# Eden-Kramer-Lab/spectral_connectivity

Hardware: AMD Instinct MI355X
Metric: channel-pair*freq-bins/s for CSM+coherence(+wPLI) (higher is better)
Workload: dtype f32

## Files before the change

### spectral_connectivity_amd/csrc/sc_api.hip

```cpp
#include <stdarg.h>
#include <stdlib.h>
#include <string.h>
#include <rocfft/rocfft.h>
#include "sc_common.h"

static thread_local char g_err[512] = "";

void sc_set_error(const char* fmt, ...) {
    va_list ap;
    va_start(ap, fmt);
    vsnprintf(g_err, sizeof(g_err), fmt, ap);
    va_end(ap);
}

static const char* const g_switch_names[SC_SW_COUNT] = {
    "SC_FUSED_DEBUG", "SC_FUSED2_TERMS", "SC_FUSED_SPLIT", "SC_FUSED_NO_SMALL", "SC_MTFFT_DEBUG", "SC_MTFFT_WIDE", "SC_MTFFT_F64",
    "SC_F64_SPLIT", "SC_F64_OC", "SC_F64_NO_FORK", "SC_F64_NO_BLOCK", "SC_WILSON_FFT", "SC_GLOBAL_EIG", "SC_GLOBAL_NT256",
    "SC_GRANGER_KERNEL", "SC_FUSED_FOLD_OBS", "SC_MTFFT_LONG", "SC_CANON_EIG", "SC_MTFFT_MIXED", "SC_MTFFT_MIXED_GEO", "SC_MTFFT_SLICE", "SC_MVAR_INVERSE"};
static char g_switch_val[SC_SW_COUNT][32];
static bool g_switch_set[SC_SW_COUNT];
extern "C" int sc_debug_reload_env(void) {
    for (int i = 0; i < SC_SW_COUNT; ++i) {
        const char* v = getenv(g_switch_names[i]);
        g_switch_set[i] = v != nullptr;
        if (v) { strncpy(g_switch_val[i], v, sizeof(g_switch_val[i]) - 1); g_switch_val[i][sizeof(g_switch_val[i]) - 1] = 0; }
    }
    return SC_OK;
}
static const int g_switches_loaded = sc_debug_reload_env();
const char* sc_switch(int id) { return (id >= 0 && id < SC_SW_COUNT && g_switch_set[id]) ? g_switch_val[id] : nullptr; }

#include <mutex>
#include <vector>
struct ScZ2zEntry { int type; size_t N, batch; rocfft_plan plan; };
static std::vector<ScZ2zEntry> g_z2z;
static std::mutex g_z2z_mutex;
static int64_t g_plans_created = 0;
int sc_internal_z2z_plan(rocfft_plan* plan, int forward, size_t N, size_t batch, bool* cached) {
    std::lock_guard<std::mutex> lock(g_z2z_mutex);
    for (const ScZ2zEntry& e : g_z2z)
        if (e.type == forward && e.N == N && e.batch == batch) { *plan = e.plan; *cached = true; return SC_OK; }
    size_t lengths[1] = {N};
    const rocfft_status s = rocfft_plan_create(plan, rocfft_placement_inplace,
                                               forward ? rocfft_transform_type_complex_forward : rocfft_transform_type_complex_inverse,
                                               rocfft_precision_double, 1, lengths, batch, nullptr);
    if (s != rocfft_status_success) {
        sc_set_error("rocfft_plan_create(Z2Z N=%zu batch=%zu) failed: %d", N, batch, (int)s);
        return SC_EFFT;
    }
    ++g_plans_created;
    *cached = true;
    g_z2z.push_back(ScZ2zEntry{forward, N, batch, *plan});
    return SC_OK;
}

struct ScR2cEntry { int64_t N, rows; int f64; rocfft_plan plan; bool busy; };
static std::vector<ScR2cEntry> g_r2c;
static rocfft_plan r2c_pool_take(int64_t N, int64_t rows, bool f64) {
    std::lock_guard<std::mutex> lock(g_z2z_mutex);
    for (ScR2cEntry& e : g_r2c)
        if (!e.busy && e.N == N && e.rows == rows && e.f64 == (f64 ? 1 : 0)) { e.busy = true; return e.plan; }
    return nullptr;
}
static void r2c_pool_add(int64_t N, int64_t rows, bool f64, rocfft_plan plan) {
    std::lock_guard<std::mutex> lock(g_z2z_mutex);
    ++g_plans_created;
    g_r2c.push_back(ScR2cEntry{N, rows, f64 ? 1 : 0, plan, true});
}
static void r2c_pool_release(rocfft_plan plan) {
    if (!plan) return;
    std::lock_guard<std::mutex> lock(g_z2z_mutex);
    for (ScR2cEntry& e : g_r2c)
        if (e.plan == plan) { e.busy = false; return; }
}
extern "C" int sc_debug_fft_plans(int64_t* n_created, int64_t* n_pooled, int64_t* n_idle) {
    std::lock_guard<std::mutex> lock(g_z2z_mutex);
    int64_t idle = 0;
    for (const ScR2cEntry& e : g_r2c) idle += e.busy ? 0 : 1;
    if (n_created) *n_created = g_plans_created;
    if (n_pooled) *n_pooled = (int64_t)(g_r2c.size() + g_z2z.size());
    if (n_idle) *n_idle = idle;
    return SC_OK;
}

extern "C" int sc_abi_version(void) { return SC_ABI_VERSION; }
extern "C" const char* sc_last_error(void) { return g_err; }

extern "C" int sc_device_count(int* count) {
    SC_REQUIRE(count != nullptr, "count is NULL");
    int n = 0;
    hipError_t e = hipGetDeviceCount(&n);
    if (e != hipSuccess) { (void)hipGetLastError(); n = 0; }
    *count = n;
    return SC_OK;
}

struct sc_fft_plan {
    rocfft_plan plan, tail_plan;
    rocfft_execution_info info;
    void* work;
    void* Z;
    size_t work_bytes;
    int64_t N, batch, chunk, tail;
    int f64;
};

static int g_rocfft_ready = 0;

#define SC_CHECK_FFT(expr)                                                          \
    do {                                                                            \
        rocfft_status s_ = (expr);                                                  \
        if (s_ != rocfft_status_success) {                                          \
            sc_set_error("%s failed: rocfft_status %d (%s:%d)", #expr, (int)s_,     \
                         __FILE__, __LINE__);                                       \
            return SC_EFFT;                                                         \
        }                                                                           \
    } while (0)

static int make_r2c_rows(rocfft_plan* plan, int64_t N, int64_t rows, bool f64) {
    if ((*plan = r2c_pool_take(N, rows, f64)) != nullptr) return SC_OK;
    rocfft_plan_description desc = nullptr;
    SC_CHECK_FFT(rocfft_plan_description_create(&desc));
    size_t one[1] = {1};
    const size_t F = (size_t)(N / 2 + 1);
    SC_CHECK_FFT(rocfft_plan_description_set_data_layout(
        desc, rocfft_array_type_real, rocfft_array_type_hermitian_interleaved, nullptr, nullptr,
        1, one, (size_t)N, 1, one, F));
    size_t lengths[1] = {(size_t)N};
    const rocfft_status s = rocfft_plan_create(plan, rocfft_placement_notinplace, rocfft_transform_type_real_forward,
                                               f64 ? rocfft_precision_double : rocfft_precision_single, 1, lengths,
                                               (size_t)rows, desc);
    rocfft_plan_description_destroy(desc);
    if (s != rocfft_status_success) {
        sc_set_error("rocfft_plan_create(N=%lld, rows=%lld) failed: status %d", (long long)N, (long long)rows, (int)s);
        *plan = nullptr;
        return SC_EFFT;
    }
    r2c_pool_add(N, rows, f64, *plan);
    return SC_OK;
}

extern "C" int sc_fft_plan_destroy(sc_fft_plan* plan);

static int fft_plan_create(sc_fft_plan** out, int64_t N, int64_t batch, bool f64) {
    SC_REQUIRE(out != nullptr, "plan out pointer is NULL");
    SC_REQUIRE(N >= 1 && batch >= 1, "N and batch must be positive");
    if (!g_rocfft_ready) { SC_CHECK_FFT(rocfft_setup()); g_rocfft_ready = 1; }
    sc_fft_plan* p = new sc_fft_plan();
    memset(p, 0, sizeof(*p));
    p->N = N; p->batch = batch; p->f64 = f64 ? 1 : 0;
    const int64_t F = N / 2 + 1;
    const size_t zsize = f64 ? sizeof(double2) : sizeof(float2);
    int64_t chunk = ((int64_t)(64u << 20) / (F * (int64_t)zsize)) & ~(int64_t)63;
    if (chunk < 64) chunk = 64;
    if (chunk > batch) chunk = batch;
    p->chunk = chunk;
    p->tail = batch % chunk;
    int rc = make_r2c_rows(&p->plan, N, chunk, f64);
    if (rc == SC_OK && p->tail) rc = make_r2c_rows(&p->tail_plan, N, p->tail, f64);
    if (rc != SC_OK) { sc_fft_plan_destroy(p); return rc; }
    size_t w1 = 0, w2 = 0;
    if (rocfft_plan_get_work_buffer_size(p->plan, &w1) != rocfft_status_success ||
        (p->tail_plan && rocfft_plan_get_work_buffer_size(p->tail_plan, &w2) != rocfft_status_success) ||
        rocfft_execution_info_create(&p->info) != rocfft_status_success) {
        sc_set_error("rocFFT work-buffer query failed (N=%lld)", (long long)N);
        sc_fft_plan_destroy(p);
        return SC_EFFT;
    }
    p->work_bytes = w1 > w2 ? w1 : w2;
    if ((p->work_bytes && hipMalloc(&p->work, p->work_bytes) != hipSuccess) ||
        hipMalloc((void**)&p->Z, (size_t)chunk * F * zsize) != hipSuccess) {
// ... 116 lines not shown
```

### spectral_connectivity_amd/csrc/sc_common.h

```cpp
#pragma once
#include <hip/hip_runtime.h>
#include <stdint.h>
#include <stdio.h>
#include "../../include/sc_hip.h"

void sc_set_error(const char* fmt, ...);

enum ScSwitch {
    SC_SW_FUSED_DEBUG, SC_SW_FUSED2_TERMS, SC_SW_FUSED_SPLIT, SC_SW_FUSED_NO_SMALL, SC_SW_MTFFT_DEBUG, SC_SW_MTFFT_WIDE,
    SC_SW_MTFFT_F64, SC_SW_F64_SPLIT, SC_SW_F64_OC, SC_SW_F64_NO_FORK, SC_SW_F64_NO_BLOCK, SC_SW_WILSON_FFT, SC_SW_GLOBAL_EIG,
    SC_SW_GLOBAL_NT256, SC_SW_GRANGER_KERNEL, SC_SW_FUSED_FOLD_OBS, SC_SW_MTFFT_LONG, SC_SW_CANON_EIG, SC_SW_MTFFT_MIXED, SC_SW_MTFFT_MIXED_GEO, SC_SW_MTFFT_SLICE, SC_SW_MVAR_INVERSE, SC_SW_COUNT
};
const char* sc_switch(int id);

int sc_internal_rows_to_bins(const void* d_Z, void* d_X, int64_t rows, int64_t F, int64_t batch, int64_t b_off,
                             int64_t nyquist_row, hipStream_t st);

bool sc_internal_mtfft_long_applies(int64_t N, int64_t C, int64_t groups);
int64_t sc_internal_mtfft_long_coverage(int64_t N, int64_t C);
int sc_internal_mtfft_long(const float* d_x, int64_t T, int64_t R, int64_t C, int64_t L, int64_t step, int64_t W, int64_t N,
                           const float* d_tapers, int64_t K, int detrend_type, const void* d_twiddles, void* d_X, void* d_P,
                           const float* d_scale, hipStream_t st);

bool sc_internal_mtfft_mix_has(int64_t N);
bool sc_internal_mtfft_mix_applies(int64_t N, int64_t C, int64_t groups);
int64_t sc_internal_mtfft_mix_coverage(int64_t N, int64_t C, bool planes);
int sc_internal_mtfft_mix(const float* d_x, int64_t T, int64_t R, int64_t C, int64_t L, int64_t step, int64_t W, int64_t N,
                          const float* d_tapers, int64_t K, int detrend_type, const void* d_twiddles, void* d_X, void* d_P,
                          const float* d_scale, hipStream_t st);

struct rocfft_plan_t;
int sc_internal_z2z_plan(struct rocfft_plan_t** plan, int forward, size_t N, size_t batch, bool* cached);

bool sc_internal_causal_fft_supported(int64_t N);
bool sc_internal_causal_fft_natural_supported(int64_t N);
int sc_internal_causal_fft_pair_natural(void* d_A, const int32_t* d_status, int64_t n_problems, int C, int64_t N,
                                        hipStream_t st);
int sc_internal_causal_fft_pair(void* d_A, const int32_t* d_status, int64_t n_problems, int C, int64_t N,
                                hipStream_t st);

bool sc_internal_granger_resident_applies(int64_t n_freq_accum, int64_t N);
int sc_internal_granger_resident(const void* d_accum, int64_t n_groups, int64_t N, int64_t C, uint32_t planes, int64_t n_obs,
                                 const int32_t* d_pairs, int64_t n_pairs, double tol, int max_iter, void* d_work, size_t work_bytes,
                                 int keep_output, double* d_out, int32_t* d_n_iter, int32_t* d_status, int32_t* h_summary,
                                 hipStream_t st);

int sc_internal_mvar_inverse(int64_t C, int64_t P, int64_t N, int64_t n_bins, const void* d_M, void* d_out, void* scratch,
                             const double* d_zero, hipStream_t st);
int sc_internal_mvar_gemm(int64_t C, int64_t n_problems, int64_t n_bins, const void* X, int64_t x_sp, int64_t x_sn,
                          const void* Y, int64_t y_sp, int64_t y_sn, void* O, int64_t o_sp, int64_t o_sn, hipStream_t st);

struct ScTimed {
    int slot;
    void* st;
    ScTimed(const char* name, void* stream);
    ~ScTimed();
    ScTimed(const ScTimed&) = delete;
    ScTimed& operator=(const ScTimed&) = delete;
};

#define SC_CHECK_HIP(expr)                                                        \
    do {                                                                          \
        hipError_t e_ = (expr);                                                   \
        if (e_ != hipSuccess) {                                                   \
            sc_set_error("%s failed: %s (%s:%d)", #expr, hipGetErrorString(e_),   \
                         __FILE__, __LINE__);                                     \
            return SC_EHIP;                                                       \
        }                                                                         \
    } while (0)

#define SC_REQUIRE(cond, msg)                                                     \
    do {                                                                          \
        if (!(cond)) {                                                            \
            sc_set_error("invalid argument: %s (%s)", msg, #cond);                \
            return SC_EINVAL;                                                     \
        }                                                                         \
    } while (0)

struct ScRec {
    const void* p;
    int f64;
    __host__ __device__ ScRec operator+(int64_t n) const { return ScRec{(const char*)p + n * (f64 ? 8 : 4), f64}; }
    __device__ double operator[](int64_t i) const {
        return f64 ? ((const double*)p)[i] : (double)((const float*)p)[i];
    }
};
__host__ inline ScRec sc_rec(const void* d_accum, uint32_t planes) { return ScRec{d_accum, (planes & SC_RECORD_F64) ? 1 : 0}; }

#define SC_TILE 16
#define SC_TILE_ELEMS 256
#define SC_MAX_SIGNALS 256

__host__ __device__ inline int sc_plane_count(uint32_t planes) {
    int n = 0;
    if (planes & SC_PLANE_CSM) n += 2;
    if (planes & SC_PLANE_ABS_IM) n += 1;
    if (planes & SC_PLANE_IM_SQ) n += 1;
    if (planes & SC_PLANE_SIGN_IM) n += 1;
    if (planes & SC_PLANE_UNIT) n += 2;
    return n;
}
__host__ __device__ inline int sc_plane_offset(uint32_t planes, uint32_t which) {
    int n = 0;
    if (which == SC_PLANE_CSM) return n;
    if (planes & SC_PLANE_CSM) n += 2;
    if (which == SC_PLANE_ABS_IM) return n;
    if (planes & SC_PLANE_ABS_IM) n += 1;
    if (which == SC_PLANE_IM_SQ) return n;
    if (planes & SC_PLANE_IM_SQ) n += 1;
    if (which == SC_PLANE_SIGN_IM) return n;
    if (planes & SC_PLANE_SIGN_IM) n += 1;
    return n;
}
__host__ __device__ inline int sc_n_blocks(int64_t C) { return (int)((C + SC_TILE - 1) / SC_TILE); }
__host__ __device__ inline int sc_n_tiles(int nb) { return nb * (nb + 1) / 2; }
__host__ __device__ inline int sc_tile_index(int bi, int bj, int nb) {
    return bi * nb - bi * (bi - 1) / 2 + (bj - bi);
}

struct ScCsmView {
    int64_t N, F, floats_per_bin;
    int NB, n_tiles, p_csm, two_sided;
    double n_obs;
};
inline int sc_csm_view(uint32_t planes, int64_t n_freq_accum, int64_t N, int64_t C, int64_t n_obs, ScCsmView* v) {
    SC_REQUIRE(planes & SC_PLANE_CSM, "accumulator record must contain SC_PLANE_CSM");
    SC_REQUIRE(n_freq_accum == N || n_freq_accum == N / 2 + 1, "accumulators must hold N or N/2+1 bins");
    SC_REQUIRE(n_obs >= 1, "n_observations must be positive");
    v->N = N; v->F = n_freq_accum;
    v->NB = sc_n_blocks(C); v->n_tiles = sc_n_tiles(v->NB);
    v->p_csm = sc_plane_offset(planes, SC_PLANE_CSM);
    v->two_sided = n_freq_accum == N ? 1 : 0;
    v->floats_per_bin = (int64_t)sc_plane_count(planes) * v->n_tiles * SC_TILE_ELEMS;
    v->n_obs = (double)n_obs;
    return SC_OK;
}
__device__ inline double2 sc_csm_two_sided(ScRec accum, const ScCsmView& v, int64_t g, int64_t n, int i, int j) {
    int64_t bin = n;
    bool conj = false;
    if (!v.two_sided && n > v.N / 2) { bin = v.N - n; conj = true; }
    const ScRec rec = accum + (g * v.F + bin) * v.floats_per_bin;
    int ti = i >> 4, tj = j >> 4, ii = i & 15, jj = j & 15;
    const bool m = (ti > tj) || (ti == tj && ii > jj);
    if (m) { int t = ti; ti = tj; tj = t; t = ii; ii = jj; jj = t; }
    const int64_t off = (int64_t)sc_tile_index(ti, tj, v.NB) * SC_TILE_ELEMS + ii * 16 + jj;
    const double re = rec[(int64_t)v.p_csm * v.n_tiles * SC_TILE_ELEMS + off] / v.n_obs;
    double im = rec[(int64_t)(v.p_csm + 1) * v.n_tiles * SC_TILE_ELEMS + off] / v.n_obs;
    if (m) im = -im;
    if (conj) im = -im;
    if (i == j) im = 0.0;
    return make_double2(re, im);
}

__device__ inline void sc_wg_cholesky(double2* L, int ld, int n, int* bad) {
    const int tid = threadIdx.x;
    for (int k = 0; k < n; ++k) {
        if (tid == 0) {
            const double d = L[k * ld + k].x;
            if (!(d > 0.0)) *bad = 1;
            L[k * ld + k] = make_double2(sqrt(d > 0.0 ? d : 1.0), 0.0);
        }
        __syncthreads();
        const double dk = L[k * ld + k].x;
        for (int i = k + 1 + tid; i < n; i += 256) {
// ... 78 lines not shown
```

### spectral_connectivity_amd/csrc/sc_mtfft_long.hip

```cpp
#include <cstdlib>
#include <type_traits>
#include "sc_common.h"
#include "sc_mtfft_bfly.h"

struct LongArgs {
    const float* x;
    const float* tapers;
    const float2* tw;
    float2* X;
    int R, C, L, step, W, K, detrend;
    int n_items;
    int g_off, g_end;
    int vec;
    unsigned char* P;
    const float* scale;
    int64_t row_bytes;
    int dbg;
};

typedef _Float16 ml_h16x2 __attribute__((ext_vector_type(2)));
typedef unsigned ml_u32x4 __attribute__((ext_vector_type(4)));
typedef unsigned ml_u32x2 __attribute__((ext_vector_type(2)));
__device__ __forceinline__ void ml_split2(float x0, float x1, unsigned& h, unsigned& m) {
    asm("v_cvt_pk_f16_f32 %0, %1, %2" : "=v"(h) : "v"(x0), "v"(x1));
    asm("v_fma_mixlo_f16 %0, %1, 1.0, -%2 op_sel_hi:[0,0,1]" : "=v"(m) : "v"(x0), "v"(h));
    asm("v_fma_mixhi_f16 %0, %1, 1.0, -%2 op_sel:[0,0,1] op_sel_hi:[0,0,1]" : "+v"(m) : "v"(x1), "v"(h));
}
template <int CTRL>
__device__ __forceinline__ void ml_quad_xchg(ml_u32x4& a, ml_u32x4& b, bool hi) {
#pragma unroll
    for (int d = 0; d < 4; ++d) {
        const unsigned give = hi ? a[d] : b[d];
        const unsigned take = (unsigned)__builtin_amdgcn_mov_dpp((int)give, CTRL, 0xf, 0xf, true);
        if (hi) a[d] = take; else b[d] = take;
    }
}

template <int LOG2N, int HT, bool PL, bool GRP = false>
__global__ void __launch_bounds__(2 * HT, HT == 512 ? 1 : 4) mtfft_long_kernel(LongArgs p) {
    constexpr int N = 1 << LOG2N;
    constexpr int THREADS = 2 * HT;
    constexpr int TPF = N / 16;
    constexpr int NF = HT / TPF;
    constexpr int CTH = 2 * NF;
    constexpr int CT = 2 * CTH;
    constexpr int ZS = N + N / 16 + 1;
    constexpr int WPF = TPF >= 64 ? TPF / 64 : 1;
    constexpr bool WAVE_LOCAL = TPF <= 64;
    constexpr bool GROUP_LOCAL = GRP && !WAVE_LOCAL;
    constexpr bool SLOT1 = WAVE_LOCAL || GROUP_LOCAL;
    constexpr int NB = SLOT1 ? 1 : 4;
    static_assert(LOG2N >= 8 && LOG2N <= 12, "256 ... 4096 samples");
    extern __shared__ __align__(16) unsigned char smem[];
    float2* zall = reinterpret_cast<float2*>(smem);
    constexpr int M = N / 256;
    float2* T2 = zall + 2 * NF * ZS;
    float2* TH = LOG2N == 12 ? T2 : T2 + 256;
    float2* TL = TH + (LOG2N == 12 ? 256 : M * 16);
    float* tap = reinterpret_cast<float*>(TL + M * 16);
    __shared__ unsigned gcnt[16];
    __shared__ int nzf[CT], nbf[CT];
    __shared__ unsigned mxc[CT];
    __shared__ double red[THREADS / 64][4];

    const int tid = threadIdx.x, half = tid / HT, ht = tid & (HT - 1), wv = tid >> 6;
    const int L = p.L, C = p.C, K = p.K;
    constexpr int LINE_CH = (PL && LOG2N <= 11) ? 32 : 16;
    constexpr int SUP = CTH >= LINE_CH ? 1 : LINE_CH / CTH;
    const bool sup = C > LINE_CH && SUP > 1 && !(p.dbg & 32);
    const int n_ct = sup ? (C + SUP * CT - 1) / (SUP * CT) * SUP : (C + CT - 1) / CT;
    int ch0[2], w, r;
    {
        const int m = blockIdx.x, xcd = m & 7, j = m >> 3, g = p.g_off + (j / n_ct) * 8 + xcd;
        if (g >= p.g_end) return;
        const int tile = j % n_ct;
#pragma unroll
        for (int h = 0; h < 2; ++h)
            ch0[h] = sup ? (tile / SUP) * (SUP * CT) + h * (SUP * CTH) + (tile % SUP) * CTH : tile * CT + h * CTH;
        w = g / p.R; r = g - w * p.R;
    }
    const int chalf = ch0[half];

    const int pf = ht / TPF, i = ht - pf * TPF;
    const int lp = 2 * (half * NF + pf);
    float2* zh = zall + half * NF * ZS;
    float2* zf = zh + pf * ZS;
    if (tid < CT) { nzf[tid] = 0; nbf[tid] = 0; mxc[tid] = 0u; }
    if (tid < 16) gcnt[tid] = 0u;
    static_assert(THREADS >= 256 + M * 16, "table fill");
    if (tid < 256) T2[tid] = p.tw[((tid >> 4) * (tid & 15)) * (N / 256)];
    else if (tid < 256 + M * 16) {
        const int e = tid - 256, t = e >> 4, x = e & 15;
        TL[e] = p.tw[t * x];
        if constexpr (LOG2N != 12) TH[e] = p.tw[16 * t * x];
    }
    for (int n = tid; n < N; n += THREADS) tap[n] = (n < L) ? p.tapers[n] : 0.f;
    const bool detr = p.detrend != SC_DETREND_NONE;
    auto pair_scale = [](unsigned mx, bool inverse) -> float {
        const unsigned E = mx >> 23;
        return (E >= 1u && E <= 253u) ? __uint_as_float((inverse ? E : 254u - E) << 23) : 1.f;
    };

    float2 xs[16];
    {
        constexpr int RS = LOG2N == 8 ? CT + 4 : CT + 2;
        constexpr int QR = CT / 4, V = CTH / 4;
        static_assert((size_t)(N / 2) * RS * 4 <= (size_t)2 * NF * ZS * 8, "tile does not fit the exchange buffers");
        float* tile = reinterpret_cast<float*>(smem);
        const int64_t RC = (int64_t)p.R * C;
        const float* xw = p.x + ((int64_t)w * p.step * p.R + r) * C;
        float4 v[2][4];
#pragma unroll
        for (int hh = 0; hh < 2; ++hh) {
#pragma unroll
            for (int it = 0; it < 4; ++it) {
                const int idx = tid + it * THREADS, row = idx / QR, q = idx - row * QR, c = ch0[q / V] + 4 * (q % V);
                const int n = hh * (N / 2) + row;
                v[hh][it] = make_float4(0.f, 0.f, 0.f, 0.f);
                if (n < L && c < C) {
                    const float* src = xw + (int64_t)n * RC + c;
                    if (p.vec && c + 3 < C) {
                        v[hh][it] = *reinterpret_cast<const float4*>(src);
                    } else {
                        v[hh][it].x = src[0];
                        if (c + 1 < C) v[hh][it].y = src[1];
                        if (c + 2 < C) v[hh][it].z = src[2];
                        if (c + 3 < C) v[hh][it].w = src[3];
                    }
                }
            }
        }
#pragma unroll
        for (int hh = 0; hh < 2; ++hh) {
            if (hh == 1) __syncthreads();
#pragma unroll
            for (int it = 0; it < 4; ++it) {
                const int idx = tid + it * THREADS, row = idx / QR, q = idx - row * QR;
                float2* d = reinterpret_cast<float2*>(tile + row * RS + 4 * q);
                d[0] = make_float2(v[hh][it].x, v[hh][it].y);
                d[1] = make_float2(v[hh][it].z, v[hh][it].w);
            }
            __syncthreads();
#pragma unroll
            for (int t = 8 * hh; t < 8 * hh + 8; ++t)
                xs[t] = *reinterpret_cast<const float2*>(tile + (i + (t - 8 * hh) * TPF) * RS + half * CTH + 2 * pf);
        }
    }
    double tsum[4] = {0.0, 0.0, 0.0, 0.0};
    if (detr) {
#pragma unroll
        for (int t = 0; t < 16; ++t) {
            const double l1 = (double)(i + t * TPF + 1);
            tsum[0] += (double)xs[t].x; tsum[1] += (double)xs[t].x * l1;
            tsum[2] += (double)xs[t].y; tsum[3] += (double)xs[t].y * l1;
        }
#pragma unroll
        for (int m = (TPF < 64 ? TPF : 64) / 2; m > 0; m >>= 1) {
#pragma unroll
            for (int e = 0; e < 4; ++e) tsum[e] += __shfl_xor(tsum[e], m);
        }
        if constexpr (WPF > 1) {
            if ((tid & 63) == 0) { red[wv][0] = tsum[0]; red[wv][1] = tsum[1]; red[wv][2] = tsum[2]; red[wv][3] = tsum[3]; }
        }
    }
    __syncthreads();
    if (detr) {
        const double n = (double)L, invL = 1.0 / n;
        const double St = (n + 1.0) * 0.5, Stt = (n + 1.0) * (2.0 * n + 1.0) / (6.0 * n), den = n * Stt - St * St;
        double ab[2][2];
#pragma unroll
        for (int ch = 0; ch < 2; ++ch) {
            double sum = tsum[2 * ch], sumt = tsum[2 * ch + 1];
            if constexpr (WPF > 1) {
                const int wv0 = (half * HT + pf * TPF) >> 6;
                sum = 0.0; sumt = 0.0;
#pragma unroll
                for (int q = 0; q < WPF; ++q) { sum += red[wv0 + q][2 * ch]; sumt += red[wv0 + q][2 * ch + 1]; }
            }
            sumt /= n;
            double a = 0.0, b;
            if (p.detrend == SC_DETREND_CONSTANT) {
                b = sum / n;
            } else {
                a = (den != 0.0) ? (n * sumt - St * sum) / den : 0.0;
                b = (sum - a * St) / n;
            }
            ab[ch][0] = a; ab[ch][1] = b;
        }
#pragma unroll
        for (int t = 0; t < 16; ++t) {
            const double tt = (double)(i + t * TPF + 1) * invL;
            const float dx = (float)((double)xs[t].x - (ab[0][0] * tt + ab[0][1]));
            const float dy = (float)((double)xs[t].y - (ab[1][0] * tt + ab[1][1]));
            const bool in = i + t * TPF < L;
            xs[t].x = in ? dx : 0.f;
            xs[t].y = in ? dy : 0.f;
        }
    }
    {
        unsigned or0 = 0u, or1 = 0u, mx0 = 0u, mx1 = 0u;
#pragma unroll
        for (int t = 0; t < 16; ++t) {
            const unsigned u0 = __float_as_uint(xs[t].x) & 0x7fffffffu, u1 = __float_as_uint(xs[t].y) & 0x7fffffffu;
            or0 |= u0; or1 |= u1;
            mx0 = mx0 > u0 ? mx0 : u0; mx1 = mx1 > u1 ? mx1 : u1;
        }
        const bool n0 = or0 != 0u, n1 = or1 != 0u, b0 = mx0 >= 0x7f800000u, b1 = mx1 >= 0x7f800000u;
        if (n0) nzf[lp] = 1;
        if (n1) nzf[lp + 1] = 1;
        if (b0) nbf[lp] = 1;
        if (b1) nbf[lp + 1] = 1;
        if (!b0 && n0) atomicMax(&mxc[lp], mx0);
        if (!b1 && n1) atomicMax(&mxc[lp + 1], mx1);
    }
    __syncthreads();
    {
        if (nbf[lp]) {
#pragma unroll
            for (int t = 0; t < 16; ++t) xs[t].x = 0.f;
        }
        if (nbf[lp + 1]) {
#pragma unroll
            for (int t = 0; t < 16; ++t) xs[t].y = 0.f;
        }
        const int c = chalf + 2 * pf;
        const float h0 = 0.5f * (PL ? (c < C ? p.scale[c] : 1.f) : pair_scale(mxc[lp], false));
        const float h1 = 0.5f * (PL ? (c + 1 < C ? p.scale[c + 1] : 1.f) : pair_scale(mxc[lp + 1], false));
#pragma unroll
        for (int t = 0; t < 16; ++t) { xs[t].x *= h0; xs[t].y *= h1; }
    }
    const int spr = ht & (NF - 1), fb = ht / NF, sl = 2 * (half * NF + spr), cs = chalf + 2 * spr;
    unsigned fl;
    {
        const bool na = nbf[sl] != 0, nb = nbf[sl + 1] != 0;
        fl = (na ? 1u : 0u) | (nb ? 2u : 0u) | ((!na && nzf[sl] == 0) ? 4u : 0u) | ((!nb && nzf[sl + 1] == 0) ? 8u : 0u);
    }
    const float ia = pair_scale(mxc[sl], true), ib = pair_scale(mxc[sl + 1], true);
    const bool vec_ok = (C % 2) == 0;
    const int64_t sF = (int64_t)p.W * p.R * K * C;
    float2* const Xi = p.X + ((int64_t)w * p.R + r) * K * C + cs + (int64_t)fb * sF;

    constexpr int TS = TPF + TPF / 16, FSTEP = HT / NF, FS = FSTEP + FSTEP / 16;
    const int kk = i & 15;
    float2* const zw1 = zf + 17 * i;
    float2* const zr = zf + i + (i >> 4);
    float2* const zw2 = zf + (((i - kk) << 4) + kk) + (i - kk);
    const float2* const zs = zh + spr * ZS + fb + (fb >> 4);
    const float2* const zm = zh + spr * ZS + (N - fb) + ((N - fb) >> 4) - 7 * FS;
    const float2* const zm0 = fb == 0 ? zh + spr * ZS : zm + 7 * FS;

    constexpr int TPT = N >= HT ? N / HT : 1;
    const float2* const t2 = T2 + kk;
    const float2* const th = TH + (i >> 4);
    const float2* const tl = TL + kk;

    unsigned epoch = 0u;
    unsigned* const gc = gcnt + half * NF + pf;
    auto group_barrier = [&]() {
        epoch += (unsigned)WPF;
        __builtin_amdgcn_fence(__ATOMIC_RELEASE, "workgroup");
        if ((tid & 63) == 0) __hip_atomic_fetch_add(gc, 1u, __ATOMIC_RELAXED, __HIP_MEMORY_SCOPE_WORKGROUP);
        while ((int)(__hip_atomic_load(gc, __ATOMIC_RELAXED, __HIP_MEMORY_SCOPE_WORKGROUP) - epoch) < 0) __builtin_amdgcn_s_sleep(1);
        __builtin_amdgcn_fence(__ATOMIC_ACQUIRE, "workgroup");
    };
#define PBAR()                                                      \
    do {                                                            \
        if constexpr (WAVE_LOCAL) {                                 \
            __builtin_amdgcn_fence(__ATOMIC_RELEASE, "wavefront");  \
            __builtin_amdgcn_wave_barrier();                        \
            __builtin_amdgcn_fence(__ATOMIC_ACQUIRE, "wavefront");  \
        } else if constexpr (GROUP_LOCAL) {                         \
            group_barrier();                                        \
        } else {                                                    \
            __syncthreads();                                        \
        }                                                           \
    } while (0)
    auto passes = [&](int k) {
        float2 a[16], o[16];
        const float* tk = SLOT1 ? tap + (k & 1) * N + i : tap + i;
        if (p.dbg & 2) {
#pragma unroll
            for (int b = 0; b < NB; ++b) __syncthreads();
            return;
        }
#pragma unroll
        for (int t = 0; t < 16; ++t) {
            const float h = tk[t * TPF];
            a[t] = make_float2(xs[t].x * h, xs[t].y * h);
        }
        dft16(a, o);
#pragma unroll
        for (int u = 0; u < 16; ++u) zw1[u] = o[u];
        PBAR();
        {
#pragma unroll
            for (int g = 0; g < 4; ++g) {
#pragma unroll
                for (int t = 4 * g; t < 4 * g + 4; ++t) {
                    const float2 v = zr[t * TS];
                    a[t] = (t == 0) ? v : cmul(v, t2[16 * t]);
                }
                __builtin_amdgcn_sched_barrier(0);
            }
            dft16(a, o);
            PBAR();
#pragma unroll
            for (int u = 0; u < 16; ++u) zw2[17 * u] = o[u];
            PBAR();
        }
        if constexpr (LOG2N == 12) {
#pragma unroll
            for (int g = 0; g < 4; ++g) {
#pragma unroll
                for (int t = 4 * g; t < 4 * g + 4; ++t) {
                    const float2 v = zr[t * TS];
                    a[t] = (t == 0) ? v : cmul(v, cmul(th[16 * t], tl[16 * t]));
                }
                __builtin_amdgcn_sched_barrier(0);
            }
            dft16(a, o);
#pragma unroll
            for (int u = 0; u < 16; ++u) zr[272 * u] = o[u];
        } else if constexpr (LOG2N == 11) {
#pragma unroll
            for (int b = 0; b < 2; ++b) {
                float2 q[8];
#pragma unroll
                for (int t = 0; t < 8; ++t) {
                    const float2 v = zr[b * TS + 272 * t];
                    q[t] = (t == 0) ? v : cmul(v, cmul(th[16 * t + b * (TPF / 16)], tl[16 * t]));
                }
                dft8r(q);
#pragma unroll
                for (int u = 0; u < 8; ++u) zr[b * TS + 272 * u] = q[u];
                __builtin_amdgcn_sched_barrier(0);
            }
        } else if constexpr (LOG2N == 10) {
#pragma unroll
            for (int b = 0; b < 4; ++b) {
                float2 q[4];
#pragma unroll
                for (int t = 0; t < 4; ++t) {
                    const float2 v = zr[b * TS + 272 * t];
                    q[t] = (t == 0) ? v : cmul(v, cmul(th[16 * t + b * (TPF / 16)], tl[16 * t]));
                }
                dft4r(q[0], q[1], q[2], q[3]);
#pragma unroll
                for (int u = 0; u < 4; ++u) zr[b * TS + 272 * u] = q[u];
            }
        } else if constexpr (LOG2N == 9) {
#pragma unroll
            for (int b = 0; b < 8; ++b) {
                const float2 u0 = zr[b * TS], u1 = cmul(zr[b * TS + 272], cmul(th[16 + b * (TPF / 16)], tl[16]));
                zr[b * TS] = make_float2(u0.x + u1.x, u0.y + u1.y);
                zr[b * TS + 272] = make_float2(u0.x - u1.x, u0.y - u1.y);
            }
        }
        __syncthreads();
    };

    auto put = [&](float2* dst, float2 u1, float2 u2) {
        float2 A = make_float2((u1.x + u2.x) * ia, (u1.y - u2.y) * ia);
        float2 B = make_float2((u1.y + u2.y) * ib, (u2.x - u1.x) * ib);
        if (fl & 4u) A = make_float2(0.f, 0.f);
        if (fl & 8u) B = make_float2(0.f, 0.f);
        if (fl & 1u) A = make_float2(__int_as_float(0x7fc00000), __int_as_float(0x7fc00000));
        if (fl & 2u) B = make_float2(__int_as_float(0x7fc00000), __int_as_float(0x7fc00000));
        if (vec_ok) {
            if (p.dbg & 16) sc_stream_store(dst, A, B);
            else *reinterpret_cast<float4*>(dst) = make_float4(A.x, A.y, B.x, B.y);
        } else {
            dst[0] = A;
            if (cs + 1 < C) dst[1] = B;
        }
    };
    constexpr int G = NF >= 4 ? 4 : NF, NG = NF / G, FSP = HT / NG, PIT = (N / 2) / FSP + 1;
#ifdef ML_QUAD_TR
    constexpr bool TR = NG >= 4;
#else
    constexpr bool TR = false;
#endif
    const int pj = ht & 3, pgrp = TR ? (ht >> 2) % NG : ht % NG, pfq = TR ? (ht / (4 * NG)) * 4 + pj : ht / NG, pcg = chalf + 2 * G * pgrp;
    bool pflag = false;
    if constexpr (PL) {
#pragma unroll
        for (int q = 0; q < 2 * G; ++q) {
            const int e = 2 * (half * NF + G * pgrp) + q;
            pflag = pflag || nbf[e] != 0 || nzf[e] == 0;
        }
        pflag = __builtin_amdgcn_ballot_w64(pflag) != 0ull;
    }
    auto put_planes = [&](int k, int it) {
        using VT = std::conditional_t<G == 4, ml_u32x4, ml_u32x2>;
        const int f = pfq + it * FSP;
        if (!(pcg < ((C + 31) & ~31)) || (TR ? f - pj : f) > N / 2) return;
        const int64_t rows_f = (int64_t)p.W * p.R * K;
        unsigned char* dst0 = p.P + (((int64_t)w * p.R + r) * K + k) * p.row_bytes + (pcg >> 5) * 256 + (pcg & 31) * 2 + (TR ? pj * 64 : 0);
        const int fr = f <= N / 2 ? f : N / 2;
        float2 u1q[G], u2q[G];
        const float2* zg = zh + (G * pgrp) * ZS;
        const int i1 = fr + (fr >> 4), n2 = (N - fr) & (N - 1), i2 = n2 + (n2 >> 4);
#pragma unroll
        for (int q = 0; q < G; ++q) { u1q[q] = zg[q * ZS + i1]; u2q[q] = zg[q * ZS + i2]; }
        VT rh, rm, ih, im;
#pragma unroll
        for (int q = 0; q < G; ++q) {
            const float2 u1 = u1q[q], u2 = u2q[q];
            float2 A = make_float2(u1.x + u2.x, u1.y - u2.y);
            float2 B = make_float2(u1.y + u2.y, u2.x - u1.x);
            if (pflag) {
                const int e = 2 * (half * NF + G * pgrp + q);
                const bool qna = nbf[e] != 0, qnb = nbf[e + 1] != 0;
                if (!qna && nzf[e] == 0) A = make_float2(0.f, 0.f);
                if (!qnb && nzf[e + 1] == 0) B = make_float2(0.f, 0.f);
                if (qna) A = make_float2(__int_as_float(0x7fc00000), __int_as_float(0x7fc00000));
                if (qnb) B = make_float2(__int_as_float(0x7fc00000), __int_as_float(0x7fc00000));
            }
            unsigned h, m;
            ml_split2(A.x, B.x, h, m);
            rh[q] = h; rm[q] = m;
            ml_split2(A.y, B.y, h, m);
            ih[q] = h; im[q] = m;
        }
        const int64_t fs = rows_f * p.row_bytes;
        if constexpr (TR) {
            ml_quad_xchg<0xB1>(rh, rm, (pj & 1) != 0);
            ml_quad_xchg<0xB1>(ih, im, (pj & 1) != 0);
            ml_quad_xchg<0x4E>(rh, ih, (pj & 2) != 0);
            ml_quad_xchg<0x4E>(rm, im, (pj & 2) != 0);
            const int f0 = f - pj;
            unsigned char* dst = dst0 + (int64_t)f0 * fs;
            *reinterpret_cast<VT*>(dst) = rh;
            if (f0 + 1 <= N / 2) *reinterpret_cast<VT*>(dst + fs) = rm;
            if (f0 + 2 <= N / 2) *reinterpret_cast<VT*>(dst + 2 * fs) = ih;
            if (f0 + 3 <= N / 2) *reinterpret_cast<VT*>(dst + 3 * fs) = im;
        } else {
            unsigned char* dst = dst0 + (int64_t)f * fs;
            *reinterpret_cast<VT*>(dst) = rh;
            *reinterpret_cast<VT*>(dst + 64) = rm;
            *reinterpret_cast<VT*>(dst + 128) = ih;
            *reinterpret_cast<VT*>(dst + 192) = im;
        }
    };
    auto store = [&](int k) {
        float2* Xk = Xi + (int64_t)k * C;
        const int64_t sR = (int64_t)FSTEP * sF;
        const bool live = cs < C && !(p.dbg & 5);
        const bool park = half == 0 && k + 1 < K;
        float hn[TPT];
        if (park) {
            const float* tp = p.tapers + ((int64_t)(k + 1) * L + ht);
#pragma unroll
            for (int j = 0; j < TPT; ++j) hn[j] = (ht + j * HT < L) ? tp[j * HT] : 0.f;
        }
#pragma unroll
        for (int ch = 0; ch < 4; ++ch) {
            if constexpr (PL) {
                if (!(p.dbg & 5)) {
#pragma unroll
                    for (int it = ch; it < (ch == 3 ? PIT : ch + 1); ++it) put_planes(k, it);
                }
            } else if (live) {
                float2 z1[2], z2[2];
#pragma unroll
                for (int it = 0; it < 2; ++it) {
                    const int m = 2 * ch + it;
                    z1[it] = zs[m * FS];
                    z2[it] = m == 0 ? zm0[0] : zm[(7 - m) * FS];
                }
#pragma unroll
                for (int it = 0; it < 2; ++it) put(Xk + (2 * ch + it) * sR, z1[it], z2[it]);
                if (ch == 3 && ht < NF) {
                    const float2 zn = zs[8 * FS];
                    put(Xk + 8 * sR, zn, zn);
                }
            }
            if constexpr (!SLOT1) __syncthreads();
            if (ch == 0 && park) {
                float* tn = SLOT1 ? tap + ((k + 1) & 1) * N : tap;
#pragma unroll
                for (int j = 0; j < TPT; ++j)
                    if (ht + j * HT < N) tn[ht + j * HT] = hn[j];
            }
        }
        if constexpr (SLOT1) __syncthreads();
    };

#pragma nounroll
    for (int gs = 0; gs <= 2 * K; ++gs) {
        const int q = gs - half;
        if (q < 0 || q >= 2 * K) {
#pragma unroll
            for (int b = 0; b < NB; ++b) __syncthreads();
        } else if (!(q & 1)) {
            passes(q >> 1);
        } else {
            store(q >> 1);
        }
    }
}

static bool long_enabled() {
    const char* e = sc_switch(SC_SW_MTFFT_LONG);
    return !e || atoi(e) != 0;
}

bool sc_internal_mtfft_long_applies(int64_t N, int64_t C, int64_t groups) {
    if (!long_enabled()) return false;
    const char* e = sc_switch(SC_SW_MTFFT_LONG);
    const bool force = e && atoi(e) == 1;
    const int lo = (e && atoi(e) >= 256) ? atoi(e) : 256;
    if (!(N >= lo && N <= 4096 && (N & (N - 1)) == 0 && C >= 1)) return false;
    if (force) return true;
    const int64_t ct = 4 * ((N <= 512 ? 256 : 512) / (N / 16));
    return groups * ((C + ct - 1) / ct) >= 256;
}

int64_t sc_internal_mtfft_long_coverage(int64_t N, int64_t C) {
    const int64_t ht = N <= 512 ? 256 : 512, nf = ht / (N / 16), ct = 4 * nf, line = N <= 2048 ? 32 : 16, sup = 2 * nf >= line ? 1 : line / (2 * nf);
    const char* d = sc_switch(SC_SW_MTFFT_DEBUG);
    const int dbg = d ? atoi(d) : 0;
    if (dbg & 64) return 0;
    return (C > line && sup > 1 && !(dbg & 32)) ? (C + sup * ct - 1) / (sup * ct) * sup * ct : (C + ct - 1) / ct * ct;
}

template <int LOG2N, int HT, bool PL, bool GRP = false>
static int launch_long_(LongArgs a, hipStream_t st) {
    constexpr int N = 1 << LOG2N, TPF = N / 16, NF = HT / TPF, CT = 4 * NF, ZS = N + N / 16 + 1;
    constexpr size_t lds = (size_t)2 * NF * ZS * 8 + (256 + (LOG2N == 12 ? 256 : 2 * (N / 256) * 16)) * 8 + (size_t)N * 4 * ((TPF <= 64 || GRP) ? 2 : 1);
    static_assert((lds + 512) * (HT == 512 ? 1 : 2) <= 160 * 1024, "LDS budget exceeded");
    auto k = mtfft_long_kernel<LOG2N, HT, PL, GRP>;
    SC_CHECK_HIP(hipFuncSetAttribute((const void*)k, hipFuncAttributeMaxDynamicSharedMemorySize, (int)lds));
    constexpr int LINE_CH = (PL && LOG2N <= 11) ? 32 : 16, SUP = 2 * NF >= LINE_CH ? 1 : LINE_CH / (2 * NF);
    const int64_t n_ct = (a.C > LINE_CH && SUP > 1 && !(a.dbg & 32)) ? (a.C + SUP * CT - 1) / (SUP * CT) * SUP : (a.C + CT - 1) / CT;
    const int64_t groups = (int64_t)a.W * a.R;
    int64_t slice_groups = groups;
    {
        const char* e = sc_switch(SC_SW_MTFFT_SLICE);
        const int64_t rounds = e ? atoll(e) : 0;
        if (rounds > 0) slice_groups = (rounds * 256 / n_ct + 7) / 8 * 8;
        if (slice_groups < 8) slice_groups = 8;
    }
    for (int64_t g0 = 0; g0 < groups; g0 += slice_groups) {
        const int64_t g1 = g0 + slice_groups < groups ? g0 + slice_groups : groups;
        const int64_t groups8 = (g1 - g0 + 7) / 8 * 8;
        if (groups8 * n_ct >= ((int64_t)1 << 31)) {
            sc_set_error("multitaper FFT (N=%d): too many windows x trials for one launch", N);
            return SC_EINVAL;
        }
        a.n_items = (int)(groups8 * n_ct);
        a.g_off = (int)g0; a.g_end = (int)g1;
        hipLaunchKernelGGL(k, dim3((unsigned)a.n_items), dim3(2 * HT), lds, st, a);
    }
    SC_CHECK_HIP(hipGetLastError());
    return SC_OK;
}

template <int LOG2N, int HT, bool GRP = false>
static int launch_long(const LongArgs& a, hipStream_t st) {
    return a.P ? launch_long_<LOG2N, HT, true, GRP>(a, st) : launch_long_<LOG2N, HT, false, GRP>(a, st);
}

int sc_internal_mtfft_long(const float* d_x, int64_t T, int64_t R, int64_t C, int64_t L, int64_t step, int64_t W, int64_t N,
                           const float* d_tapers, int64_t K, int detrend_type, const void* d_twiddles, void* d_X, void* d_P,
                           const float* d_scale, hipStream_t st) {
    LongArgs a{};
    a.x = d_x; a.tapers = d_tapers; a.tw = (const float2*)d_twiddles; a.X = (float2*)d_X;
    a.P = (unsigned char*)d_P; a.scale = d_scale; a.row_bytes = 256 * ((C + 31) / 32);
    SC_REQUIRE(!d_P || (d_scale && C % 2 == 0), "planes output needs channel scales and an even number of signals");
    a.R = (int)R; a.C = (int)C; a.L = (int)L; a.step = (int)step; a.W = (int)W; a.K = (int)K; a.detrend = detrend_type;
    a.vec = (C % 4 == 0 && ((uintptr_t)d_x & 15) == 0) ? 1 : 0;
    { const char* d = sc_switch(SC_SW_MTFFT_DEBUG); a.dbg = d ? atoi(d) : 0; }
    SC_REQUIRE((W - 1) * step + L <= T, "windows exceed the time series");
    switch (N) {
    case 256: return (a.dbg & 64) ? launch_long<8, 512>(a, st) : launch_long<8, 256>(a, st);
    case 512: return (a.dbg & 64) ? launch_long<9, 512>(a, st) : launch_long<9, 256>(a, st);
    case 1024: return (a.dbg & 64) ? launch_long<10, 256>(a, st) : launch_long<10, 512>(a, st);
    case 2048: return (a.dbg & 256) ? launch_long<11, 512>(a, st) : launch_long<11, 512, true>(a, st);
    case 4096: return launch_long<12, 512>(a, st);
    }
    return SC_EUNSUPPORTED;
}
```

Baseline: 2.704 billion.

## Prefetch next taper via direct-to-LDS loads and add opt-in CU workgroup staggering

```diff
diff --git a/spectral_connectivity_amd/csrc/sc_api.hip b/spectral_connectivity_amd/csrc/sc_api.hip
--- a/spectral_connectivity_amd/csrc/sc_api.hip
+++ b/spectral_connectivity_amd/csrc/sc_api.hip
@@ -16,7 +16,7 @@
 static const char* const g_switch_names[SC_SW_COUNT] = {
     "SC_FUSED_DEBUG", "SC_FUSED2_TERMS", "SC_FUSED_SPLIT", "SC_FUSED_NO_SMALL", "SC_MTFFT_DEBUG", "SC_MTFFT_WIDE", "SC_MTFFT_F64",
     "SC_F64_SPLIT", "SC_F64_OC", "SC_F64_NO_FORK", "SC_F64_NO_BLOCK", "SC_WILSON_FFT", "SC_GLOBAL_EIG", "SC_GLOBAL_NT256",
-    "SC_GRANGER_KERNEL", "SC_FUSED_FOLD_OBS", "SC_MTFFT_LONG", "SC_CANON_EIG", "SC_MTFFT_MIXED", "SC_MTFFT_MIXED_GEO", "SC_MTFFT_SLICE", "SC_MVAR_INVERSE"};
+    "SC_GRANGER_KERNEL", "SC_FUSED_FOLD_OBS", "SC_MTFFT_LONG", "SC_CANON_EIG", "SC_MTFFT_MIXED", "SC_MTFFT_MIXED_GEO", "SC_MTFFT_SLICE", "SC_MVAR_INVERSE", "SC_MTFFT_STAGGER"};
 static char g_switch_val[SC_SW_COUNT][32];
 static bool g_switch_set[SC_SW_COUNT];
 extern "C" int sc_debug_reload_env(void) {
diff --git a/spectral_connectivity_amd/csrc/sc_common.h b/spectral_connectivity_amd/csrc/sc_common.h
--- a/spectral_connectivity_amd/csrc/sc_common.h
+++ b/spectral_connectivity_amd/csrc/sc_common.h
@@ -9,7 +9,7 @@
 enum ScSwitch {
     SC_SW_FUSED_DEBUG, SC_SW_FUSED2_TERMS, SC_SW_FUSED_SPLIT, SC_SW_FUSED_NO_SMALL, SC_SW_MTFFT_DEBUG, SC_SW_MTFFT_WIDE,
     SC_SW_MTFFT_F64, SC_SW_F64_SPLIT, SC_SW_F64_OC, SC_SW_F64_NO_FORK, SC_SW_F64_NO_BLOCK, SC_SW_WILSON_FFT, SC_SW_GLOBAL_EIG,
-    SC_SW_GLOBAL_NT256, SC_SW_GRANGER_KERNEL, SC_SW_FUSED_FOLD_OBS, SC_SW_MTFFT_LONG, SC_SW_CANON_EIG, SC_SW_MTFFT_MIXED, SC_SW_MTFFT_MIXED_GEO, SC_SW_MTFFT_SLICE, SC_SW_MVAR_INVERSE, SC_SW_COUNT
+    SC_SW_GLOBAL_NT256, SC_SW_GRANGER_KERNEL, SC_SW_FUSED_FOLD_OBS, SC_SW_MTFFT_LONG, SC_SW_CANON_EIG, SC_SW_MTFFT_MIXED, SC_SW_MTFFT_MIXED_GEO, SC_SW_MTFFT_SLICE, SC_SW_MVAR_INVERSE, SC_SW_MTFFT_STAGGER, SC_SW_COUNT
 };
 const char* sc_switch(int id);
 
diff --git a/spectral_connectivity_amd/csrc/sc_mtfft_long.hip b/spectral_connectivity_amd/csrc/sc_mtfft_long.hip
--- a/spectral_connectivity_amd/csrc/sc_mtfft_long.hip
+++ b/spectral_connectivity_amd/csrc/sc_mtfft_long.hip
@@ -1,3 +1,4 @@
+#include <atomic>
 #include <cstdlib>
 #include <type_traits>
 #include "sc_common.h"
@@ -15,6 +16,7 @@
     unsigned char* P;
     const float* scale;
     int64_t row_bytes;
+    unsigned tag;
     int dbg;
 };
 
@@ -36,7 +38,27 @@
     }
 }
 
-template <int LOG2N, int HT, bool PL, bool GRP = false>
+constexpr int ML_CU_KEYS = 4096;
+constexpr unsigned long long ML_STAG_WAIT = 5000;
+__device__ unsigned long long g_ml_ticket[ML_CU_KEYS];
+__device__ unsigned g_ml_ready[ML_CU_KEYS];
+
+__device__ __forceinline__ unsigned ml_take(unsigned long long* c, unsigned tag) {
+    unsigned long long cur = __hip_atomic_load(c, __ATOMIC_RELAXED, __HIP_MEMORY_SCOPE_AGENT);
+    for (;;) {
+        const bool mine = (unsigned)(cur >> 32) == tag;
+        const unsigned long long nxt = mine ? cur + 1ull : ((unsigned long long)tag << 32) | 1ull;
+        if (__hip_atomic_compare_exchange_strong(c, &cur, nxt, __ATOMIC_RELAXED, __ATOMIC_RELAXED, __HIP_MEMORY_SCOPE_AGENT))
+            return mine ? (unsigned)cur : 0u;
+    }
+}
+__device__ __forceinline__ int ml_cu_key() {
+    const unsigned hw = (unsigned)__builtin_amdgcn_s_getreg((31 << 11) | (0 << 6) | 4);
+    const unsigned xcc = (unsigned)__builtin_amdgcn_s_getreg((3 << 11) | (0 << 6) | 20);
+    return (int)((((xcc & 15u) << 8) | ((hw >> 8) & 255u)) & (unsigned)(ML_CU_KEYS - 1));
+}
+
+template <int LOG2N, int HT, bool PL, bool GRP = false, bool STAG = false>
 __global__ void __launch_bounds__(2 * HT, HT == 512 ? 1 : 4) mtfft_long_kernel(LongArgs p) {
     constexpr int N = 1 << LOG2N;
     constexpr int THREADS = 2 * HT;
@@ -62,6 +84,7 @@
     __shared__ int nzf[CT], nbf[CT];
     __shared__ unsigned mxc[CT];
     __shared__ double red[THREADS / 64][4];
+    static_assert(!STAG || (HT == 256 && !GRP), "staggered workgroups: two per compute unit");
 
     const int tid = threadIdx.x, half = tid / HT, ht = tid & (HT - 1), wv = tid >> 6;
     const int L = p.L, C = p.C, K = p.K;
@@ -69,6 +92,27 @@
     constexpr int SUP = CTH >= LINE_CH ? 1 : LINE_CH / CTH;
     const bool sup = C > LINE_CH && SUP > 1 && !(p.dbg & 32);
     const int n_ct = sup ? (C + SUP * CT - 1) / (SUP * CT) * SUP : (C + CT - 1) / CT;
+    static_assert(THREADS >= 256 + M * 16, "table fill");
+    if (tid < 256) T2[tid] = p.tw[((tid >> 4) * (tid & 15)) * (N / 256)];
+    else if (tid < 256 + M * 16) {
+        const int e = tid - 256, t = e >> 4, x = e & 15;
+        TL[e] = p.tw[t * x];
+        if constexpr (LOG2N != 12) TH[e] = p.tw[16 * t * x];
+    }
+    int cu_key = 0;
+    unsigned arrival = 0u;
+    if constexpr (STAG) {
+        if (tid == 0) {
+            cu_key = ml_cu_key();
+            arrival = ml_take(&g_ml_ticket[cu_key], p.tag);
+            if (arrival == 1u) {
+                const unsigned long long t0 = __builtin_amdgcn_s_memrealtime();
+                while (__hip_atomic_load(&g_ml_ready[cu_key], __ATOMIC_RELAXED, __HIP_MEMORY_SCOPE_AGENT) != p.tag &&
+                       __builtin_amdgcn_s_memrealtime() - t0 < ML_STAG_WAIT)
+                    __builtin_amdgcn_s_sleep(8);
+            }
+        }
+    }
     int ch0[2], w, r;
     {
         const int m = blockIdx.x, xcd = m & 7, j = m >> 3, g = p.g_off + (j / n_ct) * 8 + xcd;
@@ -87,14 +131,7 @@
     float2* zf = zh + pf * ZS;
     if (tid < CT) { nzf[tid] = 0; nbf[tid] = 0; mxc[tid] = 0u; }
     if (tid < 16) gcnt[tid] = 0u;
-    static_assert(THREADS >= 256 + M * 16, "table fill");
-    if (tid < 256) T2[tid] = p.tw[((tid >> 4) * (tid & 15)) * (N / 256)];
-    else if (tid < 256 + M * 16) {
-        const int e = tid - 256, t = e >> 4, x = e & 15;
-        TL[e] = p.tw[t * x];
-        if constexpr (LOG2N != 12) TH[e] = p.tw[16 * t * x];
-    }
-    for (int n = tid; n < N; n += THREADS) tap[n] = (n < L) ? p.tapers[n] : 0.f;
+    for (int n = tid; n < (SLOT1 ? 2 : 1) * N; n += THREADS) tap[n] = (n < L) ? p.tapers[n] : 0.f;
     const bool detr = p.detrend != SC_DETREND_NONE;
     auto pair_scale = [](unsigned mx, bool inverse) -> float {
         const unsigned E = mx >> 23;
@@ -250,6 +287,25 @@
     const float2* const zm0 = fb == 0 ? zh + spr * ZS : zm + 7 * FS;
 
     constexpr int TPT = N >= HT ? N / HT : 1;
+    auto fetch_next = [&](int k) {
+        if (half != 1 || k + 1 >= K) return;
+        const uint64_t s64 = (uint64_t)(uintptr_t)(p.tapers + (int64_t)(k + 1) * L);
+        const uint64_t src = ((uint64_t)(unsigned)__builtin_amdgcn_readfirstlane((int)(s64 >> 32)) << 32) |
+                             (unsigned)__builtin_amdgcn_readfirstlane((int)(unsigned)s64);
+        float* tn = SLOT1 ? tap + ((k + 1) & 1) * N : tap;
+        const unsigned tn0 = (unsigned)(uintptr_t)(__attribute__((address_space(3))) float*)(tn + (ht & ~63));
+#pragma unroll
+        for (int j = 0; j < TPT; ++j) {
+            const int n = ht + j * HT;
+            const unsigned dst = (unsigned)__builtin_amdgcn_readfirstlane((int)(tn0 + 4u * (unsigned)(j * HT)));
+            if (n < L)
+                asm volatile("s_mov_b32 m0, %0\n\ts_nop 0\n\tglobal_load_lds_dword %1, %2"
+                             :: "s"(dst), "v"((unsigned)n * 4u), "s"(src) : "memory", "m0");
+        }
+    };
+    auto fetch_wait = [&](int k) {
+        if (half == 1 && k + 1 < K) asm volatile("s_waitcnt vmcnt(0)" ::: "memory");
+    };
     const float2* const t2 = T2 + kk;
     const float2* const th = TH + (i >> 4);
     const float2* const tl = TL + kk;
@@ -280,7 +336,11 @@
         const float* tk = SLOT1 ? tap + (k & 1) * N + i : tap + i;
         if (p.dbg & 2) {
 #pragma unroll
-            for (int b = 0; b < NB; ++b) __syncthreads();
+            for (int b = 0; b < NB; ++b) {
+                if (b == 1 || NB == 1) fetch_next(k);
+                if (b == NB - 1) fetch_wait(k);
+                __syncthreads();
+            }
             return;
         }
 #pragma unroll
@@ -292,6 +352,7 @@
 #pragma unroll
         for (int u = 0; u < 16; ++u) zw1[u] = o[u];
         PBAR();
+        fetch_next(k);
         {
 #pragma unroll
             for (int g = 0; g < 4; ++g) {
@@ -356,6 +417,7 @@
                 zr[b * TS + 272] = make_float2(u0.x - u1.x, u0.y - u1.y);
             }
         }
+        fetch_wait(k);
         __syncthreads();
     };
 
@@ -446,13 +508,6 @@
         float2* Xk = Xi + (int64_t)k * C;
         const int64_t sR = (int64_t)FSTEP * sF;
         const bool live = cs < C && !(p.dbg & 5);
-        const bool park = half == 0 && k + 1 < K;
-        float hn[TPT];
-        if (park) {
-            const float* tp = p.tapers + ((int64_t)(k + 1) * L + ht);
-#pragma unroll
-            for (int j = 0; j < TPT; ++j) hn[j] = (ht + j * HT < L) ? tp[j * HT] : 0.f;
-        }
 #pragma unroll
         for (int ch = 0; ch < 4; ++ch) {
             if constexpr (PL) {
@@ -476,15 +531,14 @@
                 }
             }
             if constexpr (!SLOT1) __syncthreads();
-            if (ch == 0 && park) {
-                float* tn = SLOT1 ? tap + ((k + 1) & 1) * N : tap;
-#pragma unroll
-                for (int j = 0; j < TPT; ++j)
-                    if (ht + j * HT < N) tn[ht + j * HT] = hn[j];
-            }
         }
         if constexpr (SLOT1) __syncthreads();
     };
+
+    if constexpr (STAG) {
+        if (tid == 0 && arrival == 0u)
+            __hip_atomic_store(&g_ml_ready[cu_key], p.tag, __ATOMIC_RELAXED, __HIP_MEMORY_SCOPE_AGENT);
+    }
 
 #pragma nounroll
     for (int gs = 0; gs <= 2 * K; ++gs) {
@@ -498,6 +552,7 @@
             store(q >> 1);
         }
     }
+#undef PBAR
 }
 
 static bool long_enabled() {
@@ -524,12 +579,12 @@
     return (C > line && sup > 1 && !(dbg & 32)) ? (C + sup * ct - 1) / (sup * ct) * sup * ct : (C + ct - 1) / ct * ct;
 }
 
-template <int LOG2N, int HT, bool PL, bool GRP = false>
+template <int LOG2N, int HT, bool PL, bool GRP = false, bool STAG = false>
 static int launch_long_(LongArgs a, hipStream_t st) {
     constexpr int N = 1 << LOG2N, TPF = N / 16, NF = HT / TPF, CT = 4 * NF, ZS = N + N / 16 + 1;
     constexpr size_t lds = (size_t)2 * NF * ZS * 8 + (256 + (LOG2N == 12 ? 256 : 2 * (N / 256) * 16)) * 8 + (size_t)N * 4 * ((TPF <= 64 || GRP) ? 2 : 1);
     static_assert((lds + 512) * (HT == 512 ? 1 : 2) <= 160 * 1024, "LDS budget exceeded");
-    auto k = mtfft_long_kernel<LOG2N, HT, PL, GRP>;
+    auto k = mtfft_long_kernel<LOG2N, HT, PL, GRP, STAG>;
     SC_CHECK_HIP(hipFuncSetAttribute((const void*)k, hipFuncAttributeMaxDynamicSharedMemorySize, (int)lds));
     constexpr int LINE_CH = (PL && LOG2N <= 11) ? 32 : 16, SUP = 2 * NF >= LINE_CH ? 1 : LINE_CH / (2 * NF);
     const int64_t n_ct = (a.C > LINE_CH && SUP > 1 && !(a.dbg & 32)) ? (a.C + SUP * CT - 1) / (SUP * CT) * SUP : (a.C + CT - 1) / CT;
@@ -550,15 +605,19 @@
         }
         a.n_items = (int)(groups8 * n_ct);
         a.g_off = (int)g0; a.g_end = (int)g1;
+        if constexpr (STAG) {
+            static std::atomic<unsigned> seq{0};
+            a.tag = seq.fetch_add(1u) + 1u;
+        }
         hipLaunchKernelGGL(k, dim3((unsigned)a.n_items), dim3(2 * HT), lds, st, a);
     }
     SC_CHECK_HIP(hipGetLastError());
     return SC_OK;
 }
 
-template <int LOG2N, int HT, bool GRP = false>
+template <int LOG2N, int HT, bool GRP = false, bool STAG = false>
 static int launch_long(const LongArgs& a, hipStream_t st) {
-    return a.P ? launch_long_<LOG2N, HT, true, GRP>(a, st) : launch_long_<LOG2N, HT, false, GRP>(a, st);
+    return a.P ? launch_long_<LOG2N, HT, true, GRP, STAG>(a, st) : launch_long_<LOG2N, HT, false, GRP, STAG>(a, st);
 }
 
 int sc_internal_mtfft_long(const float* d_x, int64_t T, int64_t R, int64_t C, int64_t L, int64_t step, int64_t W, int64_t N,
@@ -571,10 +630,12 @@
     a.R = (int)R; a.C = (int)C; a.L = (int)L; a.step = (int)step; a.W = (int)W; a.K = (int)K; a.detrend = detrend_type;
     a.vec = (C % 4 == 0 && ((uintptr_t)d_x & 15) == 0) ? 1 : 0;
     { const char* d = sc_switch(SC_SW_MTFFT_DEBUG); a.dbg = d ? atoi(d) : 0; }
+    int stag = 0;
+    { const char* e = sc_switch(SC_SW_MTFFT_STAGGER); if (e) stag = atoi(e); }
     SC_REQUIRE((W - 1) * step + L <= T, "windows exceed the time series");
     switch (N) {
-    case 256: return (a.dbg & 64) ? launch_long<8, 512>(a, st) : launch_long<8, 256>(a, st);
-    case 512: return (a.dbg & 64) ? launch_long<9, 512>(a, st) : launch_long<9, 256>(a, st);
+    case 256: return (a.dbg & 64) ? launch_long<8, 512>(a, st) : stag >= 1 ? launch_long<8, 256, false, true>(a, st) : launch_long<8, 256>(a, st);
+    case 512: return (a.dbg & 64) ? launch_long<9, 512>(a, st) : stag >= 2 ? launch_long<9, 256, false, true>(a, st) : launch_long<9, 256>(a, st);
     case 1024: return (a.dbg & 64) ? launch_long<10, 256>(a, st) : launch_long<10, 512>(a, st);
     case 2048: return (a.dbg & 256) ? launch_long<11, 512>(a, st) : launch_long<11, 512, true>(a, st);
     case 4096: return launch_long<12, 512>(a, st);
```

Result: no change. 2.725 billion (median of 6 runs) (+0.8%).
